# microsoft/MaskFlownet

Measured on NVIDIA H100. Metric: image-pairs/sec (MaskFlownet-S forward, 1024x448), higher is better.
Workload: dtype f32

## Files before the change

maskflownet_b200/csrc/conv3x3_wgmma.cu:

```cuda
#include <cstring>
#include <type_traits>

#include "mma_tiles.cuh"
#include "split_act.cuh"

namespace mfn {
namespace um {
constexpr int MT_WIDE = 128, MT_NARROW = 64;
inline int tile_width(int OW) { return OW <= MT_NARROW && tuning().conv_narrow ? MT_NARROW : MT_WIDE; }
constexpr int R = 2;
constexpr int NTHREADS = 384;
constexpr int NCONS = 8;
constexpr int NPROD = 3;
constexpr int MAX_AS = 4, MAX_WS = 24;
constexpr int RS = 2;
constexpr int BATCH = 6;
constexpr int BAR_BYTES = 1024;

__host__ __device__ inline int n_slots(int stride, int dil) { return stride == 2 ? 2 * R + 1 : (dil >= R ? 3 * R : R + 2 * dil); }
__host__ __device__ inline int row_pitch(int mt, int stride, int dil) { return stride == 2 ? 2 * mt + 1 : mt + 2 * dil; }
__host__ __device__ inline int slot_of(int r, int ky, int stride, int dil) {
  return stride == 2 ? 2 * r + ky : (dil >= R ? ky * R + r : r + ky * dil);
}
__host__ __device__ inline int tap_xoff(int mt, int kx, int stride, int dil) {
  return stride == 2 ? (kx == 1 ? 0 : (kx == 0 ? mt : mt + 1)) : kx * dil;
}
__host__ __device__ inline int band_map(int v, int n) { return v < n ? v : (v == n + 2 ? 0 : (v == n + 5 ? n - 1 : -1)); }
__host__ __device__ inline int raw_pitch(int mt) { return mt + 8; }
__host__ __device__ inline int raw_stage_bytes(int nslots, int mt) { return 16 * nslots * raw_pitch(mt) * 4; }
__host__ __device__ inline int cout_pad(int cout) { return cout <= 128 ? (cout + 15) / 16 * 16 : 256; }
__host__ __device__ inline bool fold_hi_lo(int CoutP) { return CoutP <= 64; }
__host__ __device__ inline int taps_per_stage(int CoutP) { return CoutP <= 32 ? 9 : (CoutP <= 64 ? 3 : 1); }

__device__ __forceinline__ uint64_t desc_hi(uint32_t lbo_bytes, uint32_t sbo_bytes) {
  return ((uint64_t)((lbo_bytes >> 4) & 0x3FFFu) << 16) | ((uint64_t)((sbo_bytes >> 4) & 0x3FFFu) << 32);
}
__device__ __forceinline__ void wgmma_fence() { asm volatile("wgmma.fence.sync.aligned;" ::: "memory"); }
__device__ __forceinline__ void wgmma_commit() { asm volatile("wgmma.commit_group.sync.aligned;" ::: "memory"); }
template <int N>
__device__ __forceinline__ void wgmma_wait() { asm volatile("wgmma.wait_group.sync.aligned %0;" ::"n"(N) : "memory"); }
template <int S>
__device__ __forceinline__ void fence_acc(float (&d)[S]) {
#pragma unroll
  for (int i = 0; i < S; ++i) asm volatile("" : "+f"(d[i])::"memory");
}
template <int S>
__device__ __forceinline__ void wgmma_n16(float (&d)[S], uint64_t a, uint64_t b, uint32_t scale_d) {
  static_assert(S >= 8, "accumulator too small");
  asm volatile(
      "{\n\t.reg .pred p;\n\tsetp.ne.b32 p, %10, 0;\n\t"
      "wgmma.mma_async.sync.aligned.m64n16k16.f32.bf16.bf16 {%0, %1, %2, %3, %4, %5, %6, %7}, %8, %9, p, 1, 1, 0, 0;\n\t}"
      : "+f"(d[0]), "+f"(d[1]), "+f"(d[2]), "+f"(d[3]), "+f"(d[4]), "+f"(d[5]), "+f"(d[6]), "+f"(d[7])
      : "l"(a), "l"(b), "r"(scale_d));
}
template <int S>
__device__ __forceinline__ void wgmma_n32(float (&d)[S], uint64_t a, uint64_t b, uint32_t scale_d) {
  static_assert(S >= 16, "accumulator too small");
  asm volatile(
      "{\n\t.reg .pred p;\n\tsetp.ne.b32 p, %18, 0;\n\t"
      "wgmma.mma_async.sync.aligned.m64n32k16.f32.bf16.bf16 {%0, %1, %2, %3, %4, %5, %6, %7, %8, %9, %10, %11, %12, %13, %14, %15}, %16, %17, p, 1, 1, 0, 0;\n\t}"
      : "+f"(d[0]), "+f"(d[1]), "+f"(d[2]), "+f"(d[3]), "+f"(d[4]), "+f"(d[5]), "+f"(d[6]), "+f"(d[7]), "+f"(d[8]), "+f"(d[9]), "+f"(d[10]), "+f"(d[11]), "+f"(d[12]), "+f"(d[13]), "+f"(d[14]), "+f"(d[15])
      : "l"(a), "l"(b), "r"(scale_d));
// ... 83 lines not shown
    tx = tile % tilesX;
    ty = (tile / tilesX) % tilesY;
    n = tile / (tilesX * tilesY);
  }
}
struct SplitDev {
  int in, in_g0, in_Cg;
  unsigned char* out;
  int out_Cg, out_c0;
};
struct Work {
  int tile, part, cb, ce, nh;
};
__device__ __forceinline__ Work decode_work(int w, const SplitK& sk, int nChunks) {
  Work r;
  r.nh = 0;
  if (sk.ns == 2) {
    r.nh = w & 1;
    w >>= 1;
  }
  if (sk.k <= 1 || w < sk.from) {
    r.tile = w; r.part = -1; r.cb = 0; r.ce = nChunks;
  } else {
    const int u = w - sk.from, t = u / sk.k;
    r.tile = sk.from + t;
    r.part = u - t * sk.k;
    r.cb = r.part * nChunks / sk.k;
    r.ce = (r.part + 1) * nChunks / sk.k;
  }
  return r;
}

struct SmemMap {
  int a_lo, a_stage, w_tile, w_stage, w_off, bar_off, stg_off, total, AS, WS, raw_off, raw_stage;
};
constexpr int STG_CH = 32, SPITCH = MT_WIDE + 4;
constexpr int STG_BYTES = R * STG_CH * SPITCH * 4;
__host__ __device__ inline SmemMap smem_map(int E, int CoutP, int as_wide = 3, int stg = 0, int terms = 3, int raw = 0) {
  SmemMap m;
  m.a_lo = 2 * E * 16;
  m.a_stage = terms == 1 ? m.a_lo : 2 * m.a_lo;
  m.w_tile = terms == 1 ? 32 * CoutP : 64 * CoutP;
  const int budget = 227 * 1024 - BAR_BYTES - stg - (raw ? RS * raw : 0);
  m.w_stage = taps_per_stage(CoutP) * m.w_tile;
  if (raw)
    m.AS = 2;
  else if (taps_per_stage(CoutP) > 1)
    m.AS = (4 * m.a_stage + 4 * m.w_stage <= budget) ? 4 : ((3 * m.a_stage + 3 * m.w_stage <= budget) ? 3 : 2);
  else
    m.AS = (as_wide >= 3 && 3 * m.a_stage + 8 * m.w_stage <= budget) ? 3 : 2;
  int ws = (budget - m.AS * m.a_stage) / m.w_stage;
  m.WS = ws > MAX_WS ? MAX_WS : ws;
  m.raw_off = m.AS * m.a_stage;
  m.raw_stage = raw;
  m.w_off = m.raw_off + (raw ? RS * raw : 0);
  m.bar_off = m.w_off + m.WS * m.w_stage;
  m.stg_off = m.bar_off + BAR_BYTES;
  m.total = m.stg_off + stg;
  return m;
}
}

__global__ void conv3x3_pack_wgmma_kernel(const float* __restrict__ w, unsigned char* __restrict__ packed, int Cin, int Cout,
                                          int CoutP, int nChunks16) {
  const long long total = (long long)nChunks16 * 9 * CoutP * 8;
  for (long long i = (long long)blockIdx.x * blockDim.x + threadIdx.x; i < total; i += (long long)gridDim.x * blockDim.x) {
    const int j = (int)(i & 7);
    const int f = (int)((i >> 3) % CoutP);
    const int tap = (int)((i / (8LL * CoutP)) % 9);
    const int c = (int)(i / (8LL * CoutP * 9));
    const int ch = 16 * c + 2 * j;
    float a = 0.f, b = 0.f;
    if (f < Cout) {
      if (ch < Cin) a = w[((size_t)f * Cin + ch) * 9 + tap];
      if (ch + 1 < Cin) b = w[((size_t)f * Cin + ch + 1) * 9 + tap];
    }
    uint32_t hi, lo;
    split_pair(a, b, hi, lo);
    const int wt = 64 * CoutP;
    unsigned char* tile = packed + ((size_t)c * 9 + tap) * wt;
    if (um::fold_hi_lo(CoutP)) {
      const int off = (j >> 2) * (2 * CoutP * 16) + f * 16 + (j & 3) * 4;
      *reinterpret_cast<uint32_t*>(tile + off) = hi;
      *reinterpret_cast<uint32_t*>(tile + CoutP * 16 + off) = lo;
    } else {
      const int off = (j >> 2) * (CoutP * 16) + f * 16 + (j & 3) * 4;
      *reinterpret_cast<uint32_t*>(tile + off) = hi;
      *reinterpret_cast<uint32_t*>(tile + wt / 2 + off) = lo;
    }
  }
}

template <int NW, bool FOLD, int TPS, int TERMS, int MT>
__global__ void __launch_bounds__(um::NTHREADS, 1)
    conv3x3_wgmma_kernel(const float* __restrict__ x, long long x_bs, const unsigned char* __restrict__ wpack,
                         const float* __restrict__ bias_arg, float* __restrict__ out_base, long long out_bs, int Cin, int H, int W,
                         int OH, int OW, int Cout, int CoutP, int nChunks, float slope_arg, int tilesX, int tilesY, int numWork,
                         int stride, int dil, int out_mode_arg, int ext, um::SplitK sk, um::SplitDev xs,
                         const __grid_constant__ CUtensorMap tmx, int dbg) {
  using namespace um;
  static_assert(TERMS == 1 || TERMS == 3, "one or three products per multiply-add");
  static_assert(MT == MT_WIDE || MT == MT_NARROW, "128- or 64-pixel tile rows");
  constexpr bool FOLD_ACC = FOLD && TERMS == 3;
  constexpr int P = TERMS == 1 ? 1 : 2;
  constexpr int NCOL = FOLD_ACC ? NW / 2 : NW;
  constexpr int MB = MT / 64;
  const int out_mode_k = out_mode_arg & 0xff, lin_prefix_k = out_mode_arg >> 8;
  extern __shared__ __align__(128) unsigned char smem[];
  const int nslots = n_slots(stride, dil), PW = row_pitch(MT, stride, dil), E = nslots * PW;
  const SmemMap sm = smem_map(E, CoutP, sk.as_wide, sk.stg, TERMS, xs.in == 2 ? raw_stage_bytes(nslots, MT) : 0);
  const int AS = sm.AS, WS = sm.WS;
  const uint32_t s_base = smem_u32(smem);
  const uint32_t bar0 = s_base + sm.bar_off;
  const uint32_t a_full = bar0, a_empty = bar0 + 8 * MAX_AS, w_full = bar0 + 16 * MAX_AS, w_empty = w_full + 8 * MAX_WS;
  const uint32_t r_full = w_empty + 8 * MAX_WS, r_empty = r_full + 8 * RS;

  const int tid = threadIdx.x, lane = tid & 31;
  const int warp = __shfl_sync(0xffffffffu, tid >> 5, 0);
  const size_t plane = (size_t)H * W;

  if (tid == 0) {
    for (int i = 0; i < AS; ++i) {
      mbar_init(a_full + 8 * i, xs.in == 1 ? 1 : NPROD);
      mbar_init(a_empty + 8 * i, NCONS);
    }
    for (int i = 0; i < RS; ++i) {
      mbar_init(r_full + 8 * i, 1);
      mbar_init(r_empty + 8 * i, NPROD);
    }
    for (int i = 0; i < WS; ++i) {
      mbar_init(w_full + 8 * i, 1);
      mbar_init(w_empty + 8 * i, NCONS);
    }
    asm volatile("fence.mbarrier_init.release.cluster;" ::: "memory");
  }
  __syncthreads();

  if (warp < 8) {
    const int r = warp >> 2, wq = warp & 3;
    const uint32_t a_lbo = (uint32_t)E * 16u, b_lbo = (uint32_t)(FOLD_ACC ? 2 * CoutP : CoutP) * 16u;
    uint32_t a_off[9];
#pragma unroll
    for (int tap = 0; tap < 9; ++tap)
      a_off[tap] = (uint32_t)(slot_of(r, tap / 3, stride, dil) * PW + tap_xoff(MT, tap % 3, stride, dil));
    const uint64_t dh_a = desc_hi(a_lbo, 128u), dh_b = desc_hi(b_lbo, 128u);
    uint32_t as = 0, aph = 0, ws = 0, wph = 0;
    const uint32_t a_lo16 = (uint32_t)sm.a_lo >> 4, a_stage16 = (uint32_t)sm.a_stage >> 4, s_base16 = s_base >> 4;
    const uint32_t w_base16 = (s_base + (uint32_t)sm.w_off) >> 4, w_tile16 = (uint32_t)sm.w_tile >> 4, w_half16 = w_tile16 >> 1;
// ... 282 lines not shown
        }
      }
      return;
    }
    if (dbg & 16) {
      uint32_t as = 0, aph = 0;
      bool wrapped = false;
      for (int work = blockIdx.x; work < numWork; work += gridDim.x) {
        const Work wk = decode_work(work, sk, nChunks);
        for (int c = wk.cb; c < wk.ce; ++c) {
          if (wrapped) mbar_wait(a_empty + 8 * as, aph ^ 1);
          __syncwarp();
          if (lane == 0) mbar_arrive(a_full + 8 * as);
          if (++as == (uint32_t)AS) { as = 0; aph ^= 1; wrapped = true; }
        }
      }
      return;
    }
    const int pw = warp - 9;
    const int G = (E + 31) / 32;
    const bool one_plane = Cin <= 8;
    const int nItems = one_plane ? G : 2 * G;
    const int nb = (nItems + NPROD * BATCH - 1) / (NPROD * BATCH);
    const uint32_t pw_magic = 0xFFFFFFFFu / (uint32_t)PW + 1u;
    if (one_plane) {
      for (int st = 0; st < AS; ++st)
        for (int e = pw * 32 + lane; e < E; e += NPROD * 32) {
          unsigned char* d = smem + st * sm.a_stage + (E + e) * 16;
          *reinterpret_cast<uint4*>(d) = make_uint4(0u, 0u, 0u, 0u);
          if constexpr (P == 2) *reinterpret_cast<uint4*>(d + sm.a_lo) = make_uint4(0u, 0u, 0u, 0u);
        }
    }
    if (xs.in == 2) {
      constexpr int RP = MT + 8, CP = (R + 2) * RP;
      const uint32_t raw_bytes = (uint32_t)sm.raw_stage, raw_base = s_base + (uint32_t)sm.raw_off;
      const bool issuer = warp == 9 && lane == 0;
      int i_work = blockIdx.x, i_c = 0, i_ce = 0, i_x = 0, i_y = 0, i_n = 0;
      auto i_tile = [&]() {
        if (i_work >= numWork) return;
        const Work wk = decode_work(i_work, sk, nChunks);
        int tx, ty;
        decode_tile(wk.tile, tilesX, tilesY, sk, tx, ty, i_n);
        i_c = wk.cb;
        i_ce = wk.ce;
        i_x = tx * MT - 4;
        i_y = ty * R - 1;
      };
      auto issue = [&](uint32_t slot) {
        if (i_work >= numWork) return;
        const uint32_t bar = r_full + 8 * slot;
        if (dbg & 2) {
          mbar_arrive(bar);
        } else {
          mbar_arrive_expect_tx(bar, raw_bytes);
          tma_load_4d(raw_base + slot * raw_bytes, &tmx, i_x, i_y, 16 * i_c, i_n, bar);
        }
        if (++i_c >= i_ce) {
          i_work += gridDim.x;
          i_tile();
        }
      };
      if (issuer) {
        i_tile();
        for (int s = 0; s < RS; ++s) issue((uint32_t)s);
      }
      uint32_t as = 0, aph = 0, rs = 0, rph = 0;
      bool wrapped = false;
      for (int work = blockIdx.x; work < numWork; work += gridDim.x) {
        const Work wk = decode_work(work, sk, nChunks);
        for (int c = wk.cb; c < wk.ce; ++c) {
          mbar_wait(r_full + 8 * rs, rph);
          if (wrapped) mbar_wait(a_empty + 8 * as, aph ^ 1);
          const float* raw = reinterpret_cast<const float*>(smem + sm.raw_off + rs * raw_bytes);
          unsigned char* a_st = smem + as * sm.a_stage;
#pragma unroll 2
          for (int t = pw; t < nItems; t += NPROD) {
            const int kc = one_plane ? 0 : (t & 1);
            const int e = (one_plane ? t : (t >> 1)) * 32 + lane;
            if (e >= E) continue;
            const int slot = e / (MT + 2), pe = e - slot * (MT + 2);
            const float* s = raw + 8 * kc * CP + slot * RP + pe + 3;
            float v[8];
#pragma unroll
            for (int jj = 0; jj < 8; ++jj) v[jj] = s[jj * CP];
            if constexpr (P == 1) {
              *reinterpret_cast<uint4*>(a_st + (kc * E + e) * 16) =
                  make_uint4(bf16_pair(v[0], v[1]), bf16_pair(v[2], v[3]), bf16_pair(v[4], v[5]), bf16_pair(v[6], v[7]));
            } else {
              uint4 hi, lo;
              split_pair(v[0], v[1], hi.x, lo.x);
              split_pair(v[2], v[3], hi.y, lo.y);
              split_pair(v[4], v[5], hi.z, lo.z);
              split_pair(v[6], v[7], hi.w, lo.w);
              unsigned char* dst = a_st + (kc * E + e) * 16;
              *reinterpret_cast<uint4*>(dst) = hi;
              *reinterpret_cast<uint4*>(dst + sm.a_lo) = lo;
            }
          }
          asm volatile("fence.proxy.async.shared::cta;" ::: "memory");
          __syncwarp();
          if (lane == 0) {
            mbar_arrive(a_full + 8 * as);
            mbar_arrive(r_empty + 8 * rs);
          }
          if (issuer) {
            mbar_wait(r_empty + 8 * rs, rph);
            issue(rs);
          }
          __syncwarp();
          if (++as == (uint32_t)AS) { as = 0; aph ^= 1; wrapped = true; }
          if (++rs == (uint32_t)RS) { rs = 0; rph ^= 1; }
        }
      }
      return;
    }
    int l_work = blockIdx.x, l_c = 0, l_kb = 0, l_x0 = 0, l_y0 = 0;
    const float* l_xn = x;
    int l_ce = nChunks;
    auto set_tile = [&]() {
      const Work wk = decode_work(l_work, sk, nChunks);
      l_c = wk.cb;
      l_ce = wk.ce;
      int tx, ty, n;
      decode_tile(wk.tile, tilesX, tilesY, sk, tx, ty, n);
      l_x0 = tx * MT - (ext ? 1 : 0);
      l_y0 = ty * R - (ext ? 1 : 0);
      l_xn = x + (size_t)n * x_bs;
    };
    auto advance = [&]() {
      if (++l_kb < nb) return true;
      l_kb = 0;
      if (++l_c < l_ce) return true;
      l_work += gridDim.x;
      if (l_work >= numWork) return false;
      set_tile();
      return true;
    };
    const bool s2 = stride == 2, wide = !s2 && dil >= R;
    const int ymul = s2 ? 2 : 1, ya = s2 ? -1 : -dil, yb = wide ? dil : 0, yc = wide ? 1 : 0, yd = wide ? 0 : 1;
    const int xa = s2 ? 0 : -dil;
    const uint32_t planeu = (uint32_t)plane;
    auto load_batch = [&](float (&v)[BATCH][8]) {
      const float* xc = l_xn + (size_t)(16 * l_c) * plane;
      const int ybase = ymul * l_y0 + ya, xbase = ymul * l_x0 + xa;
// ... 96 lines not shown
template <int TERMS>
__global__ void conv3x3_wgmma_reduce_kernel(um::SplitK sk, um::SplitDev xs, int RN, const float* __restrict__ bias,
                                            float* __restrict__ out, long long out_bs, int Cout, int OH, int OW, float slope,
                                            int out_mode_arg) {
  const int out_mode = out_mode_arg & 0xff, lin_prefix = out_mode_arg >> 8;
  const long long total = (long long)RN * Cout * sk.rh * OW;
  const int F = Cout >> 2;
  for (long long i = (long long)blockIdx.x * blockDim.x + threadIdx.x; i < total; i += (long long)gridDim.x * blockDim.x) {
    float s = 0.f;
    for (int p = 0; p < sk.k; ++p) s += sk.ws[(size_t)p * (size_t)sk.part_stride + (size_t)i];
    const int x = (int)(i % OW), y = sk.y_lo + (int)((i / OW) % sk.rh), f = (int)((i / ((long long)OW * sk.rh)) % Cout);
    const int n = sk.n_lo + (int)(i / ((long long)OW * sk.rh * Cout));
    if (out_mode == 0) {
      const float b = bias ? __ldg(bias + f) : 0.f;
      const float v = leaky(s + b, f < lin_prefix ? 1.f : slope);
      if (xs.out != nullptr && f >= lin_prefix)
        sa::put_one<TERMS == 1 ? 1 : 2>(xs.out, xs.out_Cg, (long long)OH * OW, n, xs.out_c0 + f - lin_prefix, (long long)y * OW + x, v);
      else
        out[(size_t)n * out_bs + ((size_t)f * OH + y) * OW + x] = v;
    } else {
      const int ph = f / F, ff = f - ph * F;
      const float b = bias ? __ldg(bias + ff) : 0.f;
      out[(size_t)n * out_bs + ((size_t)ff * (2 * OH) + (2 * y + (ph >> 1))) * (2 * OW) + 2 * x + (ph & 1)] = leaky(s + b, slope);
    }
  }
}

static um::SplitK plan_split(int N, int Cin, int H, int W, int Cout, int stride, int dil, int grid_cap) {
  using namespace um;
  (void)dil;
  const int ns = cout_pad(Cout) > 128 ? 2 : 1;
  SplitK sk = {1, 0, 0, 0, 0, 0, nullptr, 0u, 0u, 3, ns};
  const int OH = (H - 1) / stride + 1, OW = (W - 1) / stride + 1, nChunks = (Cin + 15) / 16;
  const int MT = tile_width(OW);
  const int tilesX = (OW + MT - 1) / MT, tilesY = (OH + R - 1) / R;
  const long long tiles = (long long)N * tilesX * tilesY;
  sk.from = (int)tiles;
  const int mode = tuning().conv_splitk;
  if (!mode || tiles >= (1 << 29)) return sk;
  const int sms = grid_cap > 0 && grid_cap < kNumSMs ? grid_cap : kNumSMs;
  const int kcap = mode > 1 ? mode : 32;
  if (2 * tiles * ns <= sms) {
    int k = (int)(sms / (tiles * ns));
    if (k > nChunks / 3) k = nChunks / 3;
    if (k > 8) k = 8;
    if (k > kcap) k = kcap;
    if (k >= 2) {
      sk.k = k; sk.from = 0; sk.n_lo = 0; sk.y_lo = 0; sk.rh = OH;
    }
  } else if (ns == 1 && tiles > sms) {
    const long long rounds = tiles / sms;
    long long tail = tiles - rounds * sms;
    tail = (tail + tilesX - 1) / tilesX * tilesX;
    int k = tail > 0 ? (int)(sms / tail) : 0;
    if (k > nChunks / 2) k = nChunks / 2;
    if (k > kcap) k = kcap;
    if (tail > 0 && tail <= (long long)tilesX * tilesY && rounds <= 12 && k >= 2 && nChunks >= 16 && Cout > 64) {
      sk.k = k; sk.from = (int)(tiles - tail); sk.n_lo = N - 1;
      sk.y_lo = (int)((sk.from / tilesX) % tilesY) * R;
      sk.rh = OH - sk.y_lo;
    }
  }
  if (sk.k > 1) sk.part_stride = (long long)(N - sk.n_lo) * Cout * sk.rh * OW;
  return sk;
}

long long conv3x3_wgmma_workspace_bytes(int N, int Cin, int H, int W, int Cout, int stride, int dil) {
  const um::SplitK sk = plan_split(N, Cin, H, W, Cout, stride, dil, tuning().conv_grid_cap);
  return sk.k > 1 ? sk.k * sk.part_stride * 4 : 0;
}

int conv3x3_wgmma_launch(const float* x, long long x_bs, const unsigned char* wpack, const float* bias, float* out,
                         long long out_bs, int N, int Cin, int H, int W, int Cout, int stride, int dil, int out_mode,
                         float slope, cudaStream_t st, int ext, float* ws, long long ws_bytes, const SplitIO& sio) {
  using namespace um;
  const int terms = (out_mode & MFN_CONV_BF16) ? 1 : 3;
  out_mode &= ~MFN_CONV_BF16;
  const int grow = ext == 2 ? 8 : 2 * ext;
  const int OH = stride == 2 ? (H - 1) / 2 + 1 : H + grow, OW = stride == 2 ? (W - 1) / 2 + 1 : W + grow;
  const int MT = tile_width(OW);
  SplitDev xs = {0, 0, 0, nullptr, 0, 0};
  CUtensorMap tmx;
  memset(&tmx, 0, sizeof tmx);
  if (sio.in != nullptr) {
    if (stride != 1 || ext != 0 || sio.in_c0 % 16 != 0 || (dil >= R && dil % 2 != 0) || !aligned(sio.in, 16)) return -1;
    EncodeTiledFn fn = encode_tiled_fn();
    if (fn == nullptr) return fail(MFN_ERR_UNSUPPORTED, "cuTensorMapEncodeTiled is not available from this driver");
    const int Cg = sa::groups(sio.in_C);
    const cuuint64_t dim[4] = {8, (cuuint64_t)W, (cuuint64_t)H, (cuuint64_t)N * (terms == 1 ? 1 : 2) * Cg};
    const cuuint64_t strides[3] = {16, (cuuint64_t)W * 16, (cuuint64_t)W * H * 16};
    const cuuint32_t box[4] = {8, (cuuint32_t)row_pitch(MT, 1, dil), (cuuint32_t)(dil < R ? n_slots(1, dil) : R), dil < R ? 2u : 1u};
    const cuuint32_t es[4] = {1, 1, 1, 1};
    const CUresult r = fn(&tmx, CU_TENSOR_MAP_DATA_TYPE_BFLOAT16, 4, const_cast<void*>(sio.in), dim, strides, box, es,
                          CU_TENSOR_MAP_INTERLEAVE_NONE, CU_TENSOR_MAP_SWIZZLE_NONE, CU_TENSOR_MAP_L2_PROMOTION_L2_256B,
                          CU_TENSOR_MAP_FLOAT_OOB_FILL_NONE);
    if (r != CUDA_SUCCESS) return fail(MFN_ERR_UNSUPPORTED, "cuTensorMapEncodeTiled failed (CUresult %d)", (int)r);
    xs.in = 1;
    xs.in_g0 = sio.in_c0 / 8;
    xs.in_Cg = Cg;
  }
  if (sio.out != nullptr) {
    const int lp = out_mode >> 8;
    if ((out_mode & 0xff) != 0 || ext != 0 || sio.out_c0 % 16 != 0 || (Cout - lp) % 16 != 0 || lp % 2 != 0 ||
        sio.out_c0 + Cout - lp > sio.out_C || !aligned(sio.out, 16))
      return -1;
    xs.out = static_cast<unsigned char*>(sio.out);
    xs.out_Cg = sa::groups(sio.out_C);
    xs.out_c0 = sio.out_c0;
  }
  if (Cout > 256 || (stride != 1 && !(stride == 2 && dil == 1))) return -1;
  if (ext != 0 && !((ext == 1 || ext == 2) && stride == 1 && dil == 1 && out_mode == 0)) return -1;
  if ((out_mode >> 8) != 0 && (out_mode & 0xff) != 0) return -1;
  const int CoutP = um::cout_pad(Cout), nChunks = (Cin + 15) / 16;
  const int E = n_slots(stride, dil) * row_pitch(MT, stride, dil);
  const int as_wide = tuning().conv_as == 2 ? 2 : 3;
  const bool staged = (out_mode & 0xff) == 0 && ext == 0 &&
                      (xs.out != nullptr ? (out_mode >> 8) == 0 : OW % 4 == 0 && out_bs % 4 == 0 && aligned(out, 16)) &&
                      smem_map(E, CoutP, as_wide, STG_BYTES, terms).WS >= 2;
  int raw = 0;
  if (sio.in == nullptr && tuning().conv_tma_in && stride == 1 && dil == 1 && ext == 0 && MT == MT_WIDE && W % 4 == 0 &&
      x_bs % 4 == 0 && aligned(x, 16)) {
    raw = raw_stage_bytes(n_slots(1, 1), MT);
    if (smem_map(E, CoutP, as_wide, staged ? STG_BYTES : 0, terms, raw).WS < 3) raw = 0;
  }
  if (raw) {
    EncodeTiledFn fn = encode_tiled_fn();
    if (fn == nullptr) return fail(MFN_ERR_UNSUPPORTED, "cuTensorMapEncodeTiled is not available from this driver");
    const cuuint64_t dim[4] = {(cuuint64_t)W, (cuuint64_t)H, (cuuint64_t)Cin, (cuuint64_t)N};
    const cuuint64_t strides[3] = {(cuuint64_t)W * 4, (cuuint64_t)W * H * 4, (cuuint64_t)x_bs * 4};
    const cuuint32_t box[4] = {(cuuint32_t)raw_pitch(MT), (cuuint32_t)n_slots(1, 1), 16, 1};
    const cuuint32_t es[4] = {1, 1, 1, 1};
    const CUresult r = fn(&tmx, CU_TENSOR_MAP_DATA_TYPE_FLOAT32, 4, const_cast<float*>(x), dim, strides, box, es,
                          CU_TENSOR_MAP_INTERLEAVE_NONE, CU_TENSOR_MAP_SWIZZLE_NONE, CU_TENSOR_MAP_L2_PROMOTION_L2_256B,
                          CU_TENSOR_MAP_FLOAT_OOB_FILL_NONE);
    if (r != CUDA_SUCCESS) return fail(MFN_ERR_UNSUPPORTED, "cuTensorMapEncodeTiled failed (CUresult %d)", (int)r);
    xs.in = 2;
  }
  const SmemMap sm = smem_map(E, CoutP, as_wide, staged ? STG_BYTES : 0, terms, raw);
  if (sm.WS < 2 || E * 16 > 0x3FFF * 16) return -1;
  if ((long long)H * W >= (1LL << 27)) return -1;
  const int tilesX = (OW + MT - 1) / MT, tilesY = (OH + R - 1) / R;
  const int ns = CoutP > 128 ? 2 : 1;
  SplitK sk = {1, 0, 0, 0, 0, 0, nullptr, 0u, 0u, 3, ns};
  if (ws != nullptr && ext == 0) {
    sk = plan_split(N, Cin, H, W, Cout, stride, dil, tuning().conv_grid_cap);
    if (sk.k > 1 && ws_bytes < sk.k * sk.part_stride * 4) sk.k = 1;
    sk.ws = ws;
  }
  const long long tiles = (long long)N * tilesX * tilesY;
  if (tiles * ns >= (1LL << 30)) return -1;
  sk.as_wide = as_wide;
  sk.stg = staged ? STG_BYTES : 0;
  if (sk.k <= 1) sk.from = (int)tiles;
  {
    const unsigned long long tp = (unsigned long long)tilesX * tilesY;
    if ((unsigned long long)tiles * tp < (1ull << 32) && tp * tilesX < (1ull << 32)) {
      sk.magic_tp = (uint32_t)(((1ull << 32) + tp - 1) / tp);
      sk.magic_tx = tilesX == 1 ? 0u : (uint32_t)(((1ull << 32) + tilesX - 1) / tilesX);
    }
    if (tp == 1) sk.magic_tp = 0;
  }
  const long long numWork = (sk.from + (tiles - sk.from) * sk.k) * ns;
  const int cap = tuning().conv_grid_cap > 0 ? tuning().conv_grid_cap : kNumSMs;
  const unsigned grid = (unsigned)(numWork < cap ? numWork : cap);
  const char* name = terms == 3 ? "conv3x3_wgmma_kernel<CoutP=256>" : "conv3x3_wgmma_kernel<CoutP=256,bf16>";
  auto launch = [&](auto mt) -> cudaError_t {
    constexpr int M = decltype(mt)::value;
    static SmemOptIn opt[8], opt1[8];
    cudaError_t e = cudaSuccess;
    if (terms == 3) {
      e = ensure_dyn_smem(conv3x3_wgmma_kernel<32, true, 9, 3, M>, sm.total, opt[0]);
// ... 68 lines not shown
```

maskflownet_b200/network.py:

```python
from __future__ import annotations

import math
from typing import Dict, List, Optional, Tuple

import torch
import torch.nn as nn
import torch.nn.functional as tF

from . import ops

PYRAMID_CH = {1: 16, 2: 32, 3: 64, 4: 96, 5: 128, 6: 196}
DECODER_CH = (128, 128, 96, 64, 32)
STRIDES = {6: 64, 5: 32, 4: 16, 3: 8, 2: 4}
SLOPE = 0.1
PRECISIONS = ("fp32", "bf16")


def _conv(cin, cout, k=3, s=1, p=1, d=1):
    return nn.Conv2d(cin, cout, k, s, p, d)


def msra_prelu_init_(module: nn.Module, slope: float = SLOPE, seed: Optional[int] = None) -> None:
    gen = torch.Generator().manual_seed(seed) if seed is not None else None
    for name, p in module.named_parameters():
# ... 120 lines not shown
        if not self._fast(x):
            return self._conv_act(name, x, 1.0)
        return ops.conv3x3(x, self._packed(name), conv.bias, conv.out_channels, 1.0, conv.dilation[0], bf16=self._bf16())

    def _conv_act(self, name, x, slope):
        conv = getattr(self, name)
        if (self.train_tc_forward and x.is_cuda and conv.kernel_size == (3, 3) and conv.padding == conv.dilation
                and conv.stride[0] == conv.stride[1] and conv.groups == 1):
            return ops.conv3x3_train(x, conv.weight, conv.bias, self._packed(name), slope, conv.dilation[0], conv.stride[0])
        y = conv(x)
        return y if slope == 1.0 else tF.leaky_relu(y, slope)

    def _fast(self, x):
        return self.use_tc_conv and x.is_cuda and not (torch.is_grad_enabled() and any(p.requires_grad for p in self.parameters()))

    def _pyramid(self, x, names):
        feats = []
        fast = self._fast(x)
        for lvl in range(1, 7):
            for j, sfx in enumerate(names):
                name = f"conv{lvl}{sfx}"
                conv = getattr(self, name)
                if fast:
                    x = ops.conv3x3(x, self._packed(name), conv.bias, conv.out_channels, SLOPE, 1, 2 if j == 0 else 1,
                                    bf16=self._bf16())
                else:
                    x = self._conv_act(name, x, SLOPE)
            feats.append(x)
        return feats

    def _pyramid_pair(self, im1, im2, names):
        if self._fast(im1):
            n = im1.shape[0]
            f = self._pyramid(torch.cat([im1, im2], dim=0), names)
            return [t[:n] for t in f], [t[n:] for t in f]
        return self._pyramid(im1, names), self._pyramid(im2, names)

    def _dense(self, lvl, x):
        if self._fast(x):
            return self._dense_split(lvl, x)
        for i in range(5):
            x = torch.cat([self._conv_act(f"conv{lvl}_{i}", x, SLOPE), x], dim=1)
        return x

    def _dense_split(self, lvl, base):
        N, Cb, H, W = base.shape
        front = sum(DECODER_CH)
        bf16 = self._bf16()
        act = ops.SplitAct(N, front + Cb, H, W, base.device, bf16=bf16)
        act.pack(base, front)
        nh = (2 + (1 if hasattr(self, f"pred_mask{lvl}") else 0)) if self.fuse_heads else 0
        lp = nh + nh % 2
        prefix = None
        off = front
        for i, oc in enumerate(DECODER_CH):
            assert off % 16 == 0 and (off - oc) % 16 == 0
            conv = getattr(self, f"conv{lvl}_{i}")
            if i == len(DECODER_CH) - 1 and nh:
                heads = self._head_convs(lvl, True)

                def build():
                    w = conv.weight.detach()
                    w = torch.cat([h.weight.detach()[:, oc:] for h in heads] + [w.new_zeros((lp - nh,) + w.shape[1:]), w],
                                  dim=0).contiguous()
                    b = torch.cat([torch.zeros(lp, device=w.device), conv.bias.detach()]).contiguous()
                    return ops.conv3x3_pack(w), b
                packed, b = self._packed_fn(f"conv{lvl}_4+heads", [conv.weight, conv.bias] + [h.weight for h in heads], build)
# ... 322 lines not shown
```

maskflownet_b200/ops.py:

```python
from __future__ import annotations

import ctypes
from typing import Optional, Tuple

import torch

from . import _lib
from ._lib import MaskflowError

CORR_AUTO, CORR_GENERIC, CORR_SIMT, CORR_MMA_BF16X3 = 0, 1, 2, 3
BORDER_MXNET15, BORDER_ZERO_CORNER = 0, 1


def _chk(t: Optional[torch.Tensor], name: str, optional: bool = False) -> Optional[torch.Tensor]:
    if t is None:
        if optional:
            return None
        raise MaskflowError(f"{name}: tensor required")
    if not t.is_cuda:
        raise MaskflowError(f"{name}: expected a CUDA tensor (got {t.device}); the hot path has no CPU implementation")
    if t.dtype != torch.float32:
        raise MaskflowError(f"{name}: expected float32, got {t.dtype}")
    return t.contiguous()

# ... 582 lines not shown
        slope, dilation, stride, has_bias = ctx.cfg
        if slope != 1.0:
            g = torch.where(y > 0, g, g * slope)
        gx, gw, gb = torch.ops.aten.convolution_backward(
            g.contiguous(), x, weight, [weight.shape[0]] if has_bias else None, [stride, stride], [dilation, dilation],
            [dilation, dilation], False, [0, 0], 1,
            [ctx.needs_input_grad[0], ctx.needs_input_grad[1], has_bias and ctx.needs_input_grad[2]])
        return gx, gw, (gb if has_bias else None), None, None, None, None


def conv3x3_train(x: torch.Tensor, weight: torch.Tensor, bias: Optional[torch.Tensor], packed: torch.Tensor,
                  leaky_slope: float = 0.1, dilation: int = 1, stride: int = 1) -> torch.Tensor:
    x = _chk(x, "conv3x3_train.x")
    if weight.dim() != 4 or tuple(weight.shape[2:]) != (3, 3) or weight.shape[1] != x.shape[1]:
        raise MaskflowError(f"conv3x3_train: weight {tuple(weight.shape)} does not fit x {tuple(x.shape)}")
    return _Conv3x3TrainFn.apply(x, weight, bias, packed, leaky_slope, dilation, stride)


def padded_size(H: int, W: int, resize=None):
    if resize is not None:
        return int(resize[0]), int(resize[1])
    return H + (64 - H % 64) % 64, W + (64 - W % 64) % 64


def preprocess(img1: torch.Tensor, img2: torch.Tensor, out_hw=None):
    for t, nm in ((img1, "img1"), (img2, "img2")):
        if not (t.is_cuda and t.is_contiguous() and t.dim() == 4 and t.dtype in (torch.uint8, torch.float32)):
            raise MaskflowError(f"preprocess: {nm} must be a contiguous CUDA uint8 / float32 NCHW tensor")
    if img1.shape != img2.shape or img1.dtype != img2.dtype:
        raise MaskflowError("preprocess: img1 and img2 must agree in shape and dtype")
    _no_grad_path("preprocess", img1, img2)
    N, C, H, W = img1.shape
    OH, OW = (H, W) if out_hw is None else (int(out_hw[0]), int(out_hw[1]))
    o1 = torch.empty((N, C, OH, OW), device=img1.device, dtype=torch.float32)
    o2 = torch.empty_like(o1)
    mean = torch.empty((N, C, 1, 1), device=img1.device, dtype=torch.float32)
    args = (_p(img1), _p(img2), 1 if img1.dtype == torch.uint8 else 0, _p(o1), _p(o2), _p(mean), N, C, H, W, OH, OW)
    if deterministic():
        nb = det_workspace_bytes("preprocess", N, C, H, W)
        _call("mfn_preprocess_forward_det", img1.device, *args, _p(_det_ws(nb, img1.device)), nb)
    else:
        _call("mfn_preprocess_forward", img1.device, *args)
    return o1, o2, mean


def postprocess(pred: torch.Tensor, H: int, W: int, flip_channels: bool = True, is_flow: bool = True) -> torch.Tensor:
    p = _chk(pred, "postprocess.pred")
    _no_grad_path("postprocess", p)
    N, CH, Hq, Wq = p.shape
    out = torch.empty((N, H, W, CH), device=p.device, dtype=torch.float32)
    _call("mfn_postprocess_forward", p.device, _p(p), _p(out), N, CH, Hq, Wq, int(H), int(W), 1 if flip_channels else 0,
          1 if is_flow else 0)
    return out


def flow_to_color(flow_xy: torch.Tensor, max_radius: Optional[float] = None, bgr: bool = False):
    f = _chk(flow_xy, "flow_to_color.flow_xy")
    if f.dim() not in (3, 4) or f.shape[-1] != 2:
        raise MaskflowError(f"flow_to_color: expected an (N,H,W,2) or (H,W,2) flow, got {tuple(f.shape)}")
    if max_radius is not None and not (0.0 < float(max_radius) < float("inf")):
        raise MaskflowError(f"flow_to_color: max_radius must be positive and finite, got {max_radius}")
    _no_grad_path("flow_to_color", f)
    f4 = f if f.dim() == 4 else f.unsqueeze(0)
    N, H, W, _ = f4.shape
    rgb = torch.empty((N, H, W, 3), device=f.device, dtype=torch.uint8)
    rad_max = torch.empty((N,), device=f.device, dtype=torch.float32)
    _call("mfn_flow_to_color", f.device, _p(f4), _p(rgb), _p(rad_max), N, H, W,
          float(max_radius) if max_radius is not None else 0.0, 1 if bgr else 0)
# ... 2 lines not shown
```

Measured before the change: 800.2.

## Extend TMA raw-input staging to stride-2 convs and avoid pyramid input concat

Stride-2 3x3 convolutions now use the TMA raw-input path. The tile width narrows to 64 so a 2x-wide input row box fits, eight-channel half-chunks are loaded into a deeper raw ring of up to four stages, and producers deinterleave even and odd columns when building the split bf16 operand tiles. Preprocess also allocates both images in one buffer, so the pyramid can view them as one batch without a torch.cat copy. The aim is to replace producer global loads with asynchronous bulk copies and to drop a copy kernel, at the cost of narrower tiles, more barrier round-trips per chunk, and less shared memory left for the weight ring.

```diff
diff --git a/maskflownet_b200/csrc/conv3x3_wgmma.cu b/maskflownet_b200/csrc/conv3x3_wgmma.cu
--- a/maskflownet_b200/csrc/conv3x3_wgmma.cu
+++ b/maskflownet_b200/csrc/conv3x3_wgmma.cu
@@ -7,13 +7,15 @@
 namespace mfn {
 namespace um {
 constexpr int MT_WIDE = 128, MT_NARROW = 64;
-inline int tile_width(int OW) { return OW <= MT_NARROW && tuning().conv_narrow ? MT_NARROW : MT_WIDE; }
+inline int tile_width(int OW, int stride) {
+  return tuning().conv_narrow && (OW <= MT_NARROW || (stride == 2 && tuning().conv_tma_in)) ? MT_NARROW : MT_WIDE;
+}
 constexpr int R = 2;
 constexpr int NTHREADS = 384;
 constexpr int NCONS = 8;
 constexpr int NPROD = 3;
 constexpr int MAX_AS = 4, MAX_WS = 24;
-constexpr int RS = 2;
+constexpr int MAX_RS = 4;
 constexpr int BATCH = 6;
 constexpr int BAR_BYTES = 1024;
 
@@ -26,8 +28,12 @@
   return stride == 2 ? (kx == 1 ? 0 : (kx == 0 ? mt : mt + 1)) : kx * dil;
 }
 __host__ __device__ inline int band_map(int v, int n) { return v < n ? v : (v == n + 2 ? 0 : (v == n + 5 ? n - 1 : -1)); }
-__host__ __device__ inline int raw_pitch(int mt) { return mt + 8; }
-__host__ __device__ inline int raw_stage_bytes(int nslots, int mt) { return 16 * nslots * raw_pitch(mt) * 4; }
+__host__ __device__ inline int raw_pitch(int mt, int stride) { return stride == 2 ? 2 * mt + 4 : mt + 8; }
+__host__ __device__ inline int raw_channels(int stride) { return stride == 2 ? 8 : 16; }
+__host__ __device__ inline int raw_stage_bytes(int nslots, int mt, int stride) {
+  return raw_channels(stride) * nslots * raw_pitch(mt, stride) * 4;
+}
+__host__ __device__ inline int raw_ring_max(int stride) { return stride == 2 ? MAX_RS : 2; }
 __host__ __device__ inline int cout_pad(int cout) { return cout <= 128 ? (cout + 15) / 16 * 16 : 256; }
 __host__ __device__ inline bool fold_hi_lo(int CoutP) { return CoutP <= 64; }
 __host__ __device__ inline int taps_per_stage(int CoutP) { return CoutP <= 32 ? 9 : (CoutP <= 64 ? 3 : 1); }
@@ -177,17 +183,25 @@
 }
 
 struct SmemMap {
-  int a_lo, a_stage, w_tile, w_stage, w_off, bar_off, stg_off, total, AS, WS, raw_off, raw_stage;
+  int a_lo, a_stage, w_tile, w_stage, w_off, bar_off, stg_off, total, AS, WS, raw_off, raw_stage, RS;
 };
 constexpr int STG_CH = 32, SPITCH = MT_WIDE + 4;
 constexpr int STG_BYTES = R * STG_CH * SPITCH * 4;
-__host__ __device__ inline SmemMap smem_map(int E, int CoutP, int as_wide = 3, int stg = 0, int terms = 3, int raw = 0) {
+__host__ __device__ inline SmemMap smem_map(int E, int CoutP, int as_wide = 3, int stg = 0, int terms = 3, int raw = 0,
+                                            int rs_max = 2) {
   SmemMap m;
   m.a_lo = 2 * E * 16;
   m.a_stage = terms == 1 ? m.a_lo : 2 * m.a_lo;
   m.w_tile = terms == 1 ? 32 * CoutP : 64 * CoutP;
-  const int budget = 227 * 1024 - BAR_BYTES - stg - (raw ? RS * raw : 0);
+  int budget = 227 * 1024 - BAR_BYTES - stg;
   m.w_stage = taps_per_stage(CoutP) * m.w_tile;
+  m.RS = 0;
+  if (raw) {
+    const int raw_off = (2 * m.a_stage + 127) / 128 * 128;
+    m.RS = rs_max;
+    while (m.RS > 2 && budget - raw_off - m.RS * raw < 3 * m.w_stage) --m.RS;
+    budget -= m.RS * raw + (raw_off - 2 * m.a_stage);
+  }
   if (raw)
     m.AS = 2;
   else if (taps_per_stage(CoutP) > 1)
@@ -196,9 +210,9 @@
     m.AS = (as_wide >= 3 && 3 * m.a_stage + 8 * m.w_stage <= budget) ? 3 : 2;
   int ws = (budget - m.AS * m.a_stage) / m.w_stage;
   m.WS = ws > MAX_WS ? MAX_WS : ws;
-  m.raw_off = m.AS * m.a_stage;
+  m.raw_off = raw ? (m.AS * m.a_stage + 127) / 128 * 128 : m.AS * m.a_stage;
   m.raw_stage = raw;
-  m.w_off = m.raw_off + (raw ? RS * raw : 0);
+  m.w_off = m.raw_off + m.RS * raw;
   m.bar_off = m.w_off + m.WS * m.w_stage;
   m.stg_off = m.bar_off + BAR_BYTES;
   m.total = m.stg_off + stg;
@@ -253,12 +267,13 @@
   const int out_mode_k = out_mode_arg & 0xff, lin_prefix_k = out_mode_arg >> 8;
   extern __shared__ __align__(128) unsigned char smem[];
   const int nslots = n_slots(stride, dil), PW = row_pitch(MT, stride, dil), E = nslots * PW;
-  const SmemMap sm = smem_map(E, CoutP, sk.as_wide, sk.stg, TERMS, xs.in == 2 ? raw_stage_bytes(nslots, MT) : 0);
-  const int AS = sm.AS, WS = sm.WS;
+  const SmemMap sm = smem_map(E, CoutP, sk.as_wide, sk.stg, TERMS, xs.in == 2 ? raw_stage_bytes(nslots, MT, stride) : 0,
+                              raw_ring_max(stride));
+  const int AS = sm.AS, WS = sm.WS, RS = sm.RS;
   const uint32_t s_base = smem_u32(smem);
   const uint32_t bar0 = s_base + sm.bar_off;
   const uint32_t a_full = bar0, a_empty = bar0 + 8 * MAX_AS, w_full = bar0 + 16 * MAX_AS, w_empty = w_full + 8 * MAX_WS;
-  const uint32_t r_full = w_empty + 8 * MAX_WS, r_empty = r_full + 8 * RS;
+  const uint32_t r_full = w_empty + 8 * MAX_WS, r_empty = r_full + 8 * MAX_RS;
 
   const int tid = threadIdx.x, lane = tid & 31;
   const int warp = __shfl_sync(0xffffffffu, tid >> 5, 0);
@@ -607,10 +622,12 @@
         }
     }
     if (xs.in == 2) {
-      constexpr int RP = MT + 8, CP = (R + 2) * RP;
+      const bool s2 = stride == 2;
+      const int RP = raw_pitch(MT, stride), CP = nslots * RP;
+      const int RPC = s2 && !one_plane ? 2 : 1;
       const uint32_t raw_bytes = (uint32_t)sm.raw_stage, raw_base = s_base + (uint32_t)sm.raw_off;
       const bool issuer = warp == 9 && lane == 0;
-      int i_work = blockIdx.x, i_c = 0, i_ce = 0, i_x = 0, i_y = 0, i_n = 0;
+      int i_work = blockIdx.x, i_c = 0, i_h = 0, i_ce = 0, i_x = 0, i_y = 0, i_n = 0;
       auto i_tile = [&]() {
         if (i_work >= numWork) return;
         const Work wk = decode_work(i_work, sk, nChunks);
@@ -618,8 +635,8 @@
         decode_tile(wk.tile, tilesX, tilesY, sk, tx, ty, i_n);
         i_c = wk.cb;
         i_ce = wk.ce;
-        i_x = tx * MT - 4;
-        i_y = ty * R - 1;
+        i_x = s2 ? 2 * tx * MT - 4 : tx * MT - 4;
+        i_y = s2 ? 2 * ty * R - 1 : ty * R - 1;
       };
       auto issue = [&](uint32_t slot) {
         if (i_work >= numWork) return;
@@ -628,8 +645,10 @@
           mbar_arrive(bar);
         } else {
           mbar_arrive_expect_tx(bar, raw_bytes);
-          tma_load_4d(raw_base + slot * raw_bytes, &tmx, i_x, i_y, 16 * i_c, i_n, bar);
-        }
+          tma_load_4d(raw_base + slot * raw_bytes, &tmx, i_x, i_y, 16 * i_c + 8 * i_h, i_n, bar);
+        }
+        if (++i_h < RPC) return;
+        i_h = 0;
         if (++i_c >= i_ce) {
           i_work += gridDim.x;
           i_tile();
@@ -644,47 +663,70 @@
       for (int work = blockIdx.x; work < numWork; work += gridDim.x) {
         const Work wk = decode_work(work, sk, nChunks);
         for (int c = wk.cb; c < wk.ce; ++c) {
-          mbar_wait(r_full + 8 * rs, rph);
-          if (wrapped) mbar_wait(a_empty + 8 * as, aph ^ 1);
-          const float* raw = reinterpret_cast<const float*>(smem + sm.raw_off + rs * raw_bytes);
           unsigned char* a_st = smem + as * sm.a_stage;
+          for (int h = 0; h < RPC; ++h) {
+            mbar_wait(r_full + 8 * rs, rph);
+            if (h == 0 && wrapped) mbar_wait(a_empty + 8 * as, aph ^ 1);
+            const float* raw = reinterpret_cast<const float*>(smem + sm.raw_off + rs * raw_bytes);
+            auto put = [&](int kc, int e, const float (&v)[8]) {
+              if constexpr (P == 1) {
+                *reinterpret_cast<uint4*>(a_st + (kc * E + e) * 16) =
+                    make_uint4(bf16_pair(v[0], v[1]), bf16_pair(v[2], v[3]), bf16_pair(v[4], v[5]), bf16_pair(v[6], v[7]));
+              } else {
+                uint4 hi, lo;
+                split_pair(v[0], v[1], hi.x, lo.x);
+                split_pair(v[2], v[3], hi.y, lo.y);
+                split_pair(v[4], v[5], hi.z, lo.z);
+                split_pair(v[6], v[7], hi.w, lo.w);
+                unsigned char* dst = a_st + (kc * E + e) * 16;
+                *reinterpret_cast<uint4*>(dst) = hi;
+                *reinterpret_cast<uint4*>(dst + sm.a_lo) = lo;
+              }
+            };
+            if (s2) {
+              constexpr int U = MT + 1;
+              for (int u = pw * 32 + lane; u < (2 * R + 1) * U; u += NPROD * 32) {
+                const int slot = u / U, j = u - slot * U;
+                const float* s = raw + slot * RP + 2 * j + 2;
+                float ve[8], vo[8];
+#pragma unroll
+                for (int jj = 0; jj < 8; ++jj) {
+                  const float2 p2 = *reinterpret_cast<const float2*>(s + jj * CP);
+                  ve[jj] = p2.x;
+                  vo[jj] = p2.y;
+                }
+                put(h, slot * PW + MT + j, vo);
+                if (j > 0) put(h, slot * PW + j - 1, ve);
+              }
+            } else {
 #pragma unroll 2
-          for (int t = pw; t < nItems; t += NPROD) {
-            const int kc = one_plane ? 0 : (t & 1);
-            const int e = (one_plane ? t : (t >> 1)) * 32 + lane;
-            if (e >= E) continue;
-            const int slot = e / (MT + 2), pe = e - slot * (MT + 2);
-            const float* s = raw + 8 * kc * CP + slot * RP + pe + 3;
-            float v[8];
-#pragma unroll
-            for (int jj = 0; jj < 8; ++jj) v[jj] = s[jj * CP];
-            if constexpr (P == 1) {
-              *reinterpret_cast<uint4*>(a_st + (kc * E + e) * 16) =
-                  make_uint4(bf16_pair(v[0], v[1]), bf16_pair(v[2], v[3]), bf16_pair(v[4], v[5]), bf16_pair(v[6], v[7]));
-            } else {
-              uint4 hi, lo;
-              split_pair(v[0], v[1], hi.x, lo.x);
-              split_pair(v[2], v[3], hi.y, lo.y);
-              split_pair(v[4], v[5], hi.z, lo.z);
-              split_pair(v[6], v[7], hi.w, lo.w);
-              unsigned char* dst = a_st + (kc * E + e) * 16;
-              *reinterpret_cast<uint4*>(dst) = hi;
-              *reinterpret_cast<uint4*>(dst + sm.a_lo) = lo;
+              for (int t = pw; t < nItems; t += NPROD) {
+                const int kc = one_plane ? 0 : (t & 1);
+                const int e = (one_plane ? t : (t >> 1)) * 32 + lane;
+                if (e >= E) continue;
+                const int slot = e / (MT + 2), pe = e - slot * (MT + 2);
+                const float* s = raw + 8 * kc * CP + slot * RP + pe + 3;
+                float v[8];
+#pragma unroll
+                for (int jj = 0; jj < 8; ++jj) v[jj] = s[jj * CP];
+                put(kc, e, v);
+              }
             }
-          }
-          asm volatile("fence.proxy.async.shared::cta;" ::: "memory");
-          __syncwarp();
-          if (lane == 0) {
-            mbar_arrive(a_full + 8 * as);
-            mbar_arrive(r_empty + 8 * rs);
-          }
-          if (issuer) {
-            mbar_wait(r_empty + 8 * rs, rph);
-            issue(rs);
-          }
-          __syncwarp();
+            const bool last = h == RPC - 1;
+            if (last) asm volatile("fence.proxy.async.shared::cta;" ::: "memory");
+            __syncwarp();
+            if (lane == 0) {
+              if (last) mbar_arrive(a_full + 8 * as);
+              mbar_arrive(r_empty + 8 * rs);
+            }
+            if (issuer) {
+              mbar_wait(r_empty + 8 * rs, rph);
+              issue(rs);
+            }
+            __syncwarp();
+            if (++rs == (uint32_t)RS) { rs = 0; rph ^= 1; }
+          }
           if (++as == (uint32_t)AS) { as = 0; aph ^= 1; wrapped = true; }
-          if (++rs == (uint32_t)RS) { rs = 0; rph ^= 1; }
         }
       }
       return;
@@ -847,7 +889,7 @@
   const int ns = cout_pad(Cout) > 128 ? 2 : 1;
   SplitK sk = {1, 0, 0, 0, 0, 0, nullptr, 0u, 0u, 3, ns};
   const int OH = (H - 1) / stride + 1, OW = (W - 1) / stride + 1, nChunks = (Cin + 15) / 16;
-  const int MT = tile_width(OW);
+  const int MT = tile_width(OW, stride);
   const int tilesX = (OW + MT - 1) / MT, tilesY = (OH + R - 1) / R;
   const long long tiles = (long long)N * tilesX * tilesY;
   sk.from = (int)tiles;
@@ -893,7 +935,7 @@
   out_mode &= ~MFN_CONV_BF16;
   const int grow = ext == 2 ? 8 : 2 * ext;
   const int OH = stride == 2 ? (H - 1) / 2 + 1 : H + grow, OW = stride == 2 ? (W - 1) / 2 + 1 : W + grow;
-  const int MT = tile_width(OW);
+  const int MT = tile_width(OW, stride);
   SplitDev xs = {0, 0, 0, nullptr, 0, 0};
   CUtensorMap tmx;
   memset(&tmx, 0, sizeof tmx);
@@ -933,17 +975,19 @@
                       (xs.out != nullptr ? (out_mode >> 8) == 0 : OW % 4 == 0 && out_bs % 4 == 0 && aligned(out, 16)) &&
                       smem_map(E, CoutP, as_wide, STG_BYTES, terms).WS >= 2;
   int raw = 0;
-  if (sio.in == nullptr && tuning().conv_tma_in && stride == 1 && dil == 1 && ext == 0 && MT == MT_WIDE && W % 4 == 0 &&
-      x_bs % 4 == 0 && aligned(x, 16)) {
-    raw = raw_stage_bytes(n_slots(1, 1), MT);
-    if (smem_map(E, CoutP, as_wide, staged ? STG_BYTES : 0, terms, raw).WS < 3) raw = 0;
+  const bool raw_geometry = stride == 1 ? dil == 1 && MT == MT_WIDE : MT == MT_NARROW && OW > MT_NARROW;
+  if (sio.in == nullptr && tuning().conv_tma_in && raw_geometry && ext == 0 && W % 4 == 0 && x_bs % 4 == 0 &&
+      aligned(x, 16)) {
+    raw = raw_stage_bytes(n_slots(stride, 1), MT, stride);
+    if (smem_map(E, CoutP, as_wide, staged ? STG_BYTES : 0, terms, raw, raw_ring_max(stride)).WS < 3) raw = 0;
   }
   if (raw) {
     EncodeTiledFn fn = encode_tiled_fn();
     if (fn == nullptr) return fail(MFN_ERR_UNSUPPORTED, "cuTensorMapEncodeTiled is not available from this driver");
     const cuuint64_t dim[4] = {(cuuint64_t)W, (cuuint64_t)H, (cuuint64_t)Cin, (cuuint64_t)N};
     const cuuint64_t strides[3] = {(cuuint64_t)W * 4, (cuuint64_t)W * H * 4, (cuuint64_t)x_bs * 4};
-    const cuuint32_t box[4] = {(cuuint32_t)raw_pitch(MT), (cuuint32_t)n_slots(1, 1), 16, 1};
+    const cuuint32_t box[4] = {(cuuint32_t)raw_pitch(MT, stride), (cuuint32_t)n_slots(stride, 1),
+                               (cuuint32_t)raw_channels(stride), 1};
     const cuuint32_t es[4] = {1, 1, 1, 1};
     const CUresult r = fn(&tmx, CU_TENSOR_MAP_DATA_TYPE_FLOAT32, 4, const_cast<float*>(x), dim, strides, box, es,
                           CU_TENSOR_MAP_INTERLEAVE_NONE, CU_TENSOR_MAP_SWIZZLE_NONE, CU_TENSOR_MAP_L2_PROMOTION_L2_256B,
@@ -951,7 +995,7 @@
     if (r != CUDA_SUCCESS) return fail(MFN_ERR_UNSUPPORTED, "cuTensorMapEncodeTiled failed (CUresult %d)", (int)r);
     xs.in = 2;
   }
-  const SmemMap sm = smem_map(E, CoutP, as_wide, staged ? STG_BYTES : 0, terms, raw);
+  const SmemMap sm = smem_map(E, CoutP, as_wide, staged ? STG_BYTES : 0, terms, raw, raw_ring_max(stride));
   if (sm.WS < 2 || E * 16 > 0x3FFF * 16) return -1;
   if ((long long)H * W >= (1LL << 27)) return -1;
   const int tilesX = (OW + MT - 1) / MT, tilesY = (OH + R - 1) / R;
diff --git a/maskflownet_b200/network.py b/maskflownet_b200/network.py
--- a/maskflownet_b200/network.py
+++ b/maskflownet_b200/network.py
@@ -176,7 +176,13 @@
     def _pyramid_pair(self, im1, im2, names):
         if self._fast(im1):
             n = im1.shape[0]
-            f = self._pyramid(torch.cat([im1, im2], dim=0), names)
+            if (im1.is_contiguous() and im2.is_contiguous() and im1.shape == im2.shape and im1.dtype == im2.dtype
+                    and im1.untyped_storage().data_ptr() == im2.untyped_storage().data_ptr()
+                    and im2.storage_offset() == im1.storage_offset() + im1.numel()):
+                x = im1.view(-1).as_strided((2 * im1.numel(),), (1,)).view((2 * n,) + tuple(im1.shape[1:]))
+            else:
+                x = torch.cat([im1, im2], dim=0)
+            f = self._pyramid(x, names)
             return [t[:n] for t in f], [t[n:] for t in f]
         return self._pyramid(im1, names), self._pyramid(im2, names)
 
diff --git a/maskflownet_b200/ops.py b/maskflownet_b200/ops.py
--- a/maskflownet_b200/ops.py
+++ b/maskflownet_b200/ops.py
@@ -638,8 +638,8 @@
     _no_grad_path("preprocess", img1, img2)
     N, C, H, W = img1.shape
     OH, OW = (H, W) if out_hw is None else (int(out_hw[0]), int(out_hw[1]))
-    o1 = torch.empty((N, C, OH, OW), device=img1.device, dtype=torch.float32)
-    o2 = torch.empty_like(o1)
+    pair = torch.empty((2 * N, C, OH, OW), device=img1.device, dtype=torch.float32)
+    o1, o2 = pair[:N], pair[N:]
     mean = torch.empty((N, C, 1, 1), device=img1.device, dtype=torch.float32)
     args = (_p(img1), _p(img2), 1 if img1.dtype == torch.uint8 else 0, _p(o1), _p(o2), _p(mean), N, C, H, W, OH, OW)
     if deterministic():
```

New measurement: 825.1, median of 6. 1.03x the previous value.
